# nju-websoft/MultiKE

Measured on AMD Instinct MI355X. Metric: scored triples/sec (pos+neg), higher is better.
Workload: dtype f32; 1 GPU; relation-view train step, C2-synth |E|=200000 |R|=550 dim=75 neg=25 batch=5000; n_ent=200000, n_rel=550, dim=75, neg=25, batch=5000, steps_per_epoch=184

## Files before the change

include/multike_hip.h:

```cpp
#ifndef MULTIKE_HIP_H
#define MULTIKE_HIP_H

#include <stdint.h>

#ifdef __cplusplus
extern "C" {
#endif

#define MKE_VERSION 106

#define MKE_OK 0
#define MKE_E_NULL (-1)
#define MKE_E_SHAPE (-2)
#define MKE_E_UNSUPPORTED (-3)
#define MKE_E_RANGE (-4)

#define MKE_LOSS_PARTIALS 2048

#define MKE_MAX_STRIDE 320

#define MKE_OPT_ADAGRAD 0
#define MKE_OPT_SGD 1
#define MKE_OPT_ADAM 2
#define MKE_OPT_ADADELTA 3
// ... 113 lines not shown
int mke_rows_update_multi_count(const mke_update_table* tables, int n_tables, int32_t tag, int stride, int dim,
                                int optimizer, float lr, const mke_count_job* count , void* stream);

typedef struct mke_kg_side {
  const int32_t* ent_list;
  int32_t ent_lo;
  int32_t n_ent;
  const int32_t* cand_table;
  const uint8_t* cand_valid;
  int32_t cand_k;
  const uint64_t* known_keys;
  uint64_t known_capacity;
} mke_kg_side;

int mke_neg_sample(
    const int32_t* pos_h, const int32_t* pos_r, const int32_t* pos_t, int64_t n_pos, int64_t pos_offset,
    const uint8_t* pos_kg , const mke_kg_side* sides ,
    int neg_per_pos, int max_try,
    uint32_t seed_lo, uint32_t seed_hi, uint32_t stream_id,
    int32_t* neg_h, int32_t* neg_r, int32_t* neg_t,
    void* stream);
int mke_neg_sample_at(
    const int32_t* pos_h, const int32_t* pos_r, const int32_t* pos_t, int64_t n_pos, const int32_t* pos_index,
    const uint8_t* pos_kg , const mke_kg_side* sides ,
    int neg_per_pos, int max_try,
    uint32_t seed_lo, uint32_t seed_hi, uint32_t stream_id,
    int32_t* neg_h, int32_t* neg_r, int32_t* neg_t,
    void* stream);

int mke_tripleset_build(
    const int32_t* h, const int32_t* r, const int32_t* t, int64_t n,
    uint64_t* keys, uint64_t capacity, void* stream);

int mke_tripleset_query(
    const int32_t* h, const int32_t* r, const int32_t* t, int64_t n,
    const uint64_t* keys, uint64_t capacity, uint8_t* out, void* stream);

int mke_sample_distinct(int64_t n, int batch, int n_steps, uint32_t seed_lo, uint32_t seed_hi, uint32_t stream_id,
                        int32_t* out , void* stream);

int mke_gathered_logistic_fwd_bwd(
    const float* hs, const float* rs, const float* ts, const float* ws ,
    int64_t n, int dim, int ld, int sign,
    float* gh, float* gr, float* gt,
    double* loss_partials ,
    void* stream);

int mke_gathered_alignment_fwd_bwd(
    const float* a, const float* b, int64_t n, int dim, int ld,
    float* ga, float* gb,
    double* loss_partials, void* stream);

int mke_align_fwd_bwd(
    const float* table_a, int a_normalize, const float* table_b, int b_normalize,
    int stride, int dim,
    const int32_t* ia, const int32_t* ib, int64_t n,
    float weight,
    float* grad_a , int32_t* touched_a, float* grad_b , int32_t* touched_b,
    int32_t tag,
    double* loss_partials, void* stream);

#define MKE_ALIGN_MAX_TABLES 4
#define MKE_ALIGN_MAX_TERMS 4
typedef struct mke_align_table {
  float* table; float* acc ; float* grad ; int32_t* touched;
  int64_t n_rows; int normalize;
} mke_align_table;
typedef struct mke_align_term { int a, b; float weight; } mke_align_term;
typedef struct mke_align_plan {
  mke_align_table tables[MKE_ALIGN_MAX_TABLES]; int n_tables;
  mke_align_term terms[MKE_ALIGN_MAX_TERMS]; int n_terms;
  int stride, dim;
// ... 323 lines not shown
```

multike_amd/_lib.py:

```python
from __future__ import annotations

import ctypes as C
import os

import numpy as np
import torch

_HERE = os.path.dirname(os.path.abspath(__file__))
SO_PATH = os.path.join(_HERE, "libmultike_hip.so")

LOSS_PARTIALS = 2048
MAX_STRIDE = 320
OPT_ADAGRAD, OPT_SGD, OPT_ADAM, OPT_ADADELTA = 0, 1, 2, 3
DENSE_OPTS = {"Adam": OPT_ADAM, "Adadelta": OPT_ADADELTA}
_SUPPORTED_FPL = (1, 2, 3, 4, 5, 6, 7, 8, 10, 12, 13, 16, 20)

SYMBOLS = (
    "mke_version", "mke_last_error", "mke_set_option", "mke_triple_score_fwd_bwd", "mke_triple_score_fwd_bwd_x",
    "mke_count_entity_refs", "mke_triple_score_fwd_bwd_xc", "mke_triple_score_fwd_bwd_xch", "mke_triple_score_fwd_bwd_det", "mke_stage_reduce", "mke_rows_update", "mke_rows_update_multi", "mke_rows_update_multi_count",
    "mke_neg_sample", "mke_tripleset_build", "mke_tripleset_query", "mke_gathered_logistic_fwd_bwd",
    "mke_gathered_alignment_fwd_bwd", "mke_align_fwd_bwd", "mke_gather_rows", "mke_relation_steps",
    "mke_rowset_build", "mke_rowset_remap", "mke_rows_gather_padded", "mke_rows_scatter_add",
    "mke_attr_conv_fwd", "mke_attr_conv_bwd", "mke_attr_tail_z", "mke_attr_tail_loss", "mke_attr_tail_bwd",
    "mke_dense_update", "mke_align_rank", "mke_gemm_f32", "mke_attr_scratch_floats", "mke_attr_step", "mke_attr_steps", "mke_attr_step_phases",
    "mke_sample_distinct", "mke_neg_sample_at", "mke_rows_update_dense", "mke_dense_update_opt", "mke_align_steps", "mke_sim_select", "mke_sim_sample", "mke_topk_rows", "mke_topk_candidates", "mke_mapping_scratch_floats", "mke_mapping_step", "mke_mapping_step_phases", "mke_mapping_steps",
    "mke_ae_scratch_floats", "mke_ae_train_steps", "mke_ae_step_phases", "mke_ae_encode", "mke_dense_layer_fwd",
    "mke_topk_long", "mke_probe_rows", "mke_oc_block_floats", "mke_oc_pack_codes", "mke_oc_plan", "mke_oc_bases", "mke_oc_count", "mke_oc_score", "mke_oc_apply", "mke_oc_run",
    "mke_oc_em_plan_temp_bytes", "mke_oc_em_plan", "mke_oc_pass2", "mke_oc_steps",
    "mke_tuning_init", "mke_triple_score_fwd_bwd_t", "mke_rows_update_multi_t",
    "mke_align_topk_mean_temp_bytes", "mke_align_topk_mean", "mke_align_rank_ex",
)
ACT_NONE, ACT_TANH, ACT_SIGMOID = 0, 1, 2
AE_MAX_LAYERS = 4


class AttrStepArgs(C.Structure):
    _fields_ = [
        ("ent_table", C.c_void_p), ("n_ent", C.c_int64), ("ent_stride", C.c_int), ("ent_normalize", C.c_int),
        ("ent_acc", C.c_void_p), ("ent_grad", C.c_void_p), ("ent_touched", C.c_void_p),
        ("attr_table", C.c_void_p), ("n_attr", C.c_int64), ("attr_stride", C.c_int), ("attr_normalize", C.c_int),
        ("attr_acc", C.c_void_p), ("attr_grad", C.c_void_p), ("attr_touched", C.c_void_p),
        ("lit_table", C.c_void_p), ("lit_stride", C.c_int), ("dim", C.c_int),
        ("ih", C.c_void_p), ("ia", C.c_void_p), ("iv", C.c_void_p), ("weights", C.c_void_p), ("n", C.c_int64),
        ("scale", C.c_float), ("params", C.c_void_p), ("param_grads", C.c_void_p), ("param_acc", C.c_void_p),
        ("scratch", C.c_void_p), ("partials", C.c_void_p), ("optimizer", C.c_int), ("lr", C.c_float), ("tag", C.c_int32),
        ("update", C.c_int), ("workspace", C.c_void_p), ("attr_grad_copies", C.c_int), ("tuning", C.c_void_p),
    ]


class AlignTableStruct(C.Structure):
    _fields_ = [("table", C.c_void_p), ("acc", C.c_void_p), ("grad", C.c_void_p), ("touched", C.c_void_p), ("n_rows", C.c_int64),
                ("normalize", C.c_int)]


class AlignTermStruct(C.Structure):
    _fields_ = [("a", C.c_int), ("b", C.c_int), ("weight", C.c_float)]


class AlignPlanStruct(C.Structure):
    _fields_ = [("tables", AlignTableStruct * 4), ("n_tables", C.c_int), ("terms", AlignTermStruct * 4), ("n_terms", C.c_int),
                ("stride", C.c_int), ("dim", C.c_int), ("ia", C.c_void_p), ("ib", C.c_void_p),
                ("step_off", C.POINTER(C.c_int64)), ("n_steps", C.c_int), ("optimizer", C.c_int), ("lr", C.c_float),
                ("tag_base", C.c_int32), ("loss_partials", C.c_void_p)]
# ... 133 lines not shown
        ("neg_per_pos", C.c_int), ("max_try", C.c_int), ("sample_chunk", C.c_int), ("negatives_ready", C.c_int),
        ("neg_h", C.c_void_p), ("neg_r", C.c_void_p), ("neg_t", C.c_void_p),
        ("seed_lo", C.c_uint32), ("seed_hi", C.c_uint32), ("stream_id", C.c_uint32),
        ("optimizer", C.c_int), ("lr", C.c_float), ("scale", C.c_float),
        ("loss_partials", C.c_void_p), ("loss_ring", C.c_int), ("tag_base", C.c_int32), ("pos_w", C.c_void_p),
        ("hot", HotRowsStruct), ("tuning", C.c_void_p),
    ]

_lib = None


class MultiKEHipError(RuntimeError):
    pass


def lib():
    global _lib
    if _lib is None:
        if not os.path.exists(SO_PATH):
            raise MultiKEHipError(
                f"{SO_PATH} not found: build it with `python -c 'import __graft_entry__ as g; g.build()'` "
                "or `make -C multike_amd/csrc`.  multike_amd has no CPU fallback.")
        L = C.CDLL(SO_PATH)
        L.mke_version.restype = C.c_int
        L.mke_last_error.restype = C.c_char_p
        for name in SYMBOLS[2:]:
            getattr(L, name).restype = C.c_int
        L.mke_attr_scratch_floats.restype = C.c_int64
        L.mke_mapping_scratch_floats.restype = C.c_int64
        L.mke_ae_scratch_floats.restype = C.c_int64
        L.mke_oc_block_floats.restype = C.c_int64
        L.mke_oc_em_plan_temp_bytes.restype = C.c_int64
        L.mke_align_topk_mean_temp_bytes.restype = C.c_int64
        _lib = L
        for kv in filter(None, os.environ.get("MKE_OPTIONS", "").split(",")):
            k, _, v = kv.partition("=")
            if L.mke_set_option(k.strip().encode(), C.c_int(int(v)), None):
                raise MultiKEHipError(f"MKE_OPTIONS: {L.mke_last_error().decode()}")
    return _lib


def stride_for(dim: int) -> int:
    need = (dim + 15) // 16
    for f in _SUPPORTED_FPL:
        if f >= need:
            return f * 16
    raise MultiKEHipError(f"dim {dim} exceeds the largest supported stride {MAX_STRIDE}")


def _check(rc: int, what: str):
    if rc != 0:
        msg = lib().mke_last_error().decode("utf-8", "replace")
        raise MultiKEHipError(f"{what} failed (code {rc}): {msg}")


def _dev(t: torch.Tensor | None, dtype, name: str):
    if t is None:
        return C.c_void_p(0)
    if not t.is_cuda:
        raise MultiKEHipError(f"{name}: expected a CUDA/HIP tensor, got device {t.device} (no CPU path exists)")
    if t.dtype != dtype:
        raise MultiKEHipError(f"{name}: expected dtype {dtype}, got {t.dtype}")
    if not t.is_contiguous():
        raise MultiKEHipError(f"{name}: tensor must be contiguous")
    return C.c_void_p(t.data_ptr())

# ... 294 lines not shown
    rc = lib().mke_mapping_step_phases(C.byref(args), _dev(loss_partials, torch.float64, "loss_partials"), C.c_int(phases), _stream())
    _check(rc, "mke_mapping_step_phases")


def mapping_step(args: MappingStepArgs, loss_partials: torch.Tensor):
    rc = lib().mke_mapping_step(C.byref(args), _dev(loss_partials, torch.float64, "loss_partials"), _stream())
    _check(rc, "mke_mapping_step")


def mapping_steps(args: MappingStepArgs, step_off: np.ndarray, loss_ring: torch.Tensor):
    off = np.ascontiguousarray(step_off, dtype=np.int64)
    rc = lib().mke_mapping_steps(C.byref(args), off.ctypes.data_as(C.POINTER(C.c_int64)), C.c_int(len(off) - 1),
                                 _dev(loss_ring, torch.float64, "loss_ring"), C.c_int(loss_ring.shape[0]), _stream())
    _check(rc, "mke_mapping_steps")


def align_steps(plan: AlignPlanStruct):
    rc = lib().mke_align_steps(C.byref(plan), _stream())
    _check(rc, "mke_align_steps")


def relation_steps(plan: RelationPlanStruct, step_begin: int, step_end: int):
    rc = lib().mke_relation_steps(C.byref(plan), C.c_int(step_begin), C.c_int(step_end), _stream())
    _check(rc, "mke_relation_steps")


def tripleset_build(h, r, t, keys):
    rc = lib().mke_tripleset_build(_dev(h, torch.int32, "h"), _dev(r, torch.int32, "r"), _dev(t, torch.int32, "t"),
                                   C.c_int64(h.numel()), _dev(keys, torch.int64, "keys"), C.c_uint64(keys.numel()),
                                   _stream())
    _check(rc, "mke_tripleset_build")


def tripleset_query(h, r, t, keys, out):
    rc = lib().mke_tripleset_query(_dev(h, torch.int32, "h"), _dev(r, torch.int32, "r"), _dev(t, torch.int32, "t"),
                                   C.c_int64(h.numel()), _dev(keys, torch.int64, "keys"), C.c_uint64(keys.numel()),
                                   _dev(out, torch.uint8, "out"), _stream())
    _check(rc, "mke_tripleset_query")


def gathered_logistic_fwd_bwd(hs, rs, ts, ws, sign, gh, gr, gt, loss_partials):
    n, dim = hs.shape
    rc = lib().mke_gathered_logistic_fwd_bwd(
        _dev(hs, torch.float32, "hs"), _dev(rs, torch.float32, "rs"), _dev(ts, torch.float32, "ts"),
        _dev(ws, torch.float32, "ws"), C.c_int64(n), C.c_int(dim), C.c_int(dim), C.c_int(sign),
        _dev(gh, torch.float32, "gh"), _dev(gr, torch.float32, "gr"), _dev(gt, torch.float32, "gt"),
        _dev(loss_partials, torch.float64, "loss_partials"), _stream())
    _check(rc, "mke_gathered_logistic_fwd_bwd")


def gathered_alignment_fwd_bwd(a, b, ga, gb, loss_partials):
    n, dim = a.shape
    rc = lib().mke_gathered_alignment_fwd_bwd(
        _dev(a, torch.float32, "a"), _dev(b, torch.float32, "b"), C.c_int64(n), C.c_int(dim), C.c_int(dim),
        _dev(ga, torch.float32, "ga"), _dev(gb, torch.float32, "gb"),
        _dev(loss_partials, torch.float64, "loss_partials"), _stream())
    _check(rc, "mke_gathered_alignment_fwd_bwd")


def align_fwd_bwd(table_a, a_normalize, table_b, b_normalize, dim, ia, ib, weight, grad_a, touched_a, grad_b, touched_b,
                  tag, loss_partials):
    rc = lib().mke_align_fwd_bwd(
        _dev(table_a, torch.float32, "table_a"), C.c_int(int(a_normalize)), _dev(table_b, torch.float32, "table_b"),
        C.c_int(int(b_normalize)), C.c_int(table_a.shape[1]), C.c_int(dim), _dev(ia, torch.int32, "ia"),
        _dev(ib, torch.int32, "ib"), C.c_int64(ia.numel()), C.c_float(weight), _dev(grad_a, torch.float32, "grad_a"),
        _dev(touched_a, torch.int32, "touched_a"), _dev(grad_b, torch.float32, "grad_b"),
# ... 360 lines not shown
```

multike_amd/csrc/mke_sampler.hip:

```cpp
#include "mke_common.h"

namespace mke {

struct SampleParams {
  const int32_t* __restrict__ ph;
  const int32_t* __restrict__ pr;
  const int32_t* __restrict__ pt;
  const uint8_t* __restrict__ pos_kg;
  int64_t n_pos, pos_offset;
  const int32_t* __restrict__ pos_index;
  int npp, max_try;
  mke_kg_side side[2];
  uint32_t seed_lo, seed_hi, sid;
  int32_t* __restrict__ nh;
  int32_t* __restrict__ nr;
  int32_t* __restrict__ nt;
};

__host__ __device__ __forceinline__ uint32_t draw_next(uint32_t gi, uint32_t round, uint32_t slot, uint32_t sid,
                                                       uint32_t k0, uint32_t k1, uint32_t n, uint32_t& attempt) {
  for (;;) {
    const uint32_t blk = attempt >> 2, word = attempt & 3u;
    const Philox4 ph = philox4x32_10(gi, round | (blk << 8), slot, sid, k0, k1);
    const uint32_t x = ph.v[word];
    ++attempt;
    const uint64_t m = (uint64_t)x * (uint64_t)n;
    const uint32_t l = (uint32_t)m;
    if (l < n) {
      const uint32_t thresh = (0u - n) % n;
      if (l < thresh) continue;
    }
    return (uint32_t)(m >> 32);
  }
}

__device__ __forceinline__ bool set_contains(const uint64_t* __restrict__ keys, uint64_t cap, uint64_t key) {
  uint64_t slot = mix64(key) & (cap - 1);
  for (;;) {
    const uint64_t k = keys[slot];
    if (k == key) return true;
    if (k == MKE_EMPTY_KEY) return false;
    slot = (slot + 1) & (cap - 1);
  }
}

template <int GS, bool FAST>
__global__ __launch_bounds__(MKE_BLOCK) void k_neg_sample(const SampleParams p) {
  constexpr int PPW = 64 / GS;
  constexpr int TS = 2 * GS;
  __shared__ uint32_t s_dup[FAST ? (MKE_BLOCK / GS) * TS : 1];
  const int lane = threadIdx.x & 63;
  const int gl = lane & (GS - 1);
  const int gbase = lane & ~(GS - 1);
  const int64_t wave = ((int64_t)blockIdx.x * MKE_BLOCK + threadIdx.x) >> 6;
  const int64_t i = wave * PPW + (lane / GS);
  const bool live = i < p.n_pos;
  const int64_t ii = live ? i : 0;
  const int h = p.ph[ii], r = p.pr[ii], t = p.pt[ii];
  const int kg = p.pos_kg ? (p.pos_kg[ii] != 0) : 0;
  const mke_kg_side& sd = p.side[kg];
  const uint32_t sid = p.sid + (uint32_t)kg;
  const uint64_t* __restrict__ keys = sd.known_keys;
  const uint32_t gi = p.pos_index ? (uint32_t)p.pos_index[ii] : (uint32_t)(ii + p.pos_offset);
  const int N = p.npp;
  const uint64_t gmask_all = GS == 64 ? ~0ull : (((1ull << (GS & 63)) - 1ull) << gbase);
  int collected = live ? 0 : N;
  for (int round = 0; round < p.max_try; ++round) {
    if (!__ballot(collected < N)) break;
    const int need = N - collected;
    const bool active = gl < need;
    const bool merged = FAST && N < GS;
    bool corrupt_head;
    uint32_t first_word = 0;
    if (merged) {
      const Philox4 ph = philox4x32_10(gi, (uint32_t)round, gl == GS - 1 ? 0xFFFFFFFFu : (uint32_t)gl, sid, p.seed_lo, p.seed_hi);
      first_word = ph.v[0];
      corrupt_head = ((uint32_t)__shfl((int)ph.v[0], gbase + GS - 1, 64) >> 31) != 0;
    } else {
      const Philox4 cph = philox4x32_10(gi, (uint32_t)round, 0xFFFFFFFFu, sid, p.seed_lo, p.seed_hi);
      corrupt_head = (cph.v[0] >> 31) != 0;
    }
    const int x = corrupt_head ? h : t;
    const bool use_tbl = sd.cand_table != nullptr && (sd.cand_valid == nullptr || sd.cand_valid[x] != 0);
    const uint32_t n = use_tbl ? (uint32_t)sd.cand_k : (uint32_t)sd.n_ent;
    uint32_t attempt = 0;
    uint32_t pos = 0xFFFFFFFFu;
    if (active) {
      bool have = false;
      if (merged) {
        attempt = 1;
        const uint64_t m = (uint64_t)first_word * (uint64_t)n;
        const uint32_t l = (uint32_t)m;
        have = l >= n || l >= (0u - n) % n;
        pos = (uint32_t)(m >> 32);
      }
// ... 11 lines not shown
        for (;;) {
          const uint32_t old = atomicCAS(&tbl[sl], 0xFFFFFFFFu, pos);
          if (old == 0xFFFFFFFFu) break;
          if (old == pos) { dup = true; break; }
          sl = (sl + 1) & (TS - 1);
        }
      }
    } else {
      for (int q = 0; q < need_max; ++q) {
        const uint32_t v = (uint32_t)__shfl((int)pos, gbase + q, 64);
        dup |= active && q < need && gl > q && pos == v;
      }
    }
    if (__ballot(dup)) {
      for (int q = 1; q < need_max; ++q) {
        for (;;) {
          const uint32_t v = (uint32_t)__shfl((int)pos, gbase + q, 64);
          const bool hit = q < need && gl < q && pos == v;
          const uint64_t hb = __ballot(hit);
          if (!hb) break;
          if ((hb & gmask_all) && gl == q) pos = draw_next(gi, (uint32_t)round, (uint32_t)gl, sid, p.seed_lo, p.seed_hi, n, attempt);
        }
      }
    }
    int ent = 0;
    if (active) {
      ent = use_tbl ? sd.cand_table[(int64_t)x * sd.cand_k + pos]
                    : (sd.ent_list ? sd.ent_list[pos] : sd.ent_lo + (int32_t)pos);
    }
    const int nh = corrupt_head ? ent : h;
    const int nt = corrupt_head ? t : ent;
    bool keep = active;
    if (active && round < p.max_try - 1 && keys != nullptr) {
      keep = !set_contains(keys, sd.known_capacity, triple_key((uint32_t)nh, (uint32_t)r, (uint32_t)nt));
    }
    const uint64_t mask = (__ballot(keep) & gmask_all) >> gbase;
    if (keep) {
      const int rank = __popcll(mask & ((1ull << gl) - 1ull));
      const int64_t o = i * (int64_t)N + collected + rank;
      p.nh[o] = nh; p.nr[o] = r; p.nt[o] = nt;
    }
    collected += __popcll(mask);
  }
}

__global__ __launch_bounds__(MKE_BLOCK) void k_tripleset_build(const int32_t* __restrict__ h, const int32_t* __restrict__ r,
                                                               const int32_t* __restrict__ t, int64_t n,
                                                               uint64_t* __restrict__ keys, uint64_t cap) {
  const int64_t i = (int64_t)blockIdx.x * MKE_BLOCK + threadIdx.x;
  if (i >= n) return;
  const uint64_t key = triple_key((uint32_t)h[i], (uint32_t)r[i], (uint32_t)t[i]);
  uint64_t slot = mix64(key) & (cap - 1);
  for (;;) {
    const unsigned long long prev =
        atomicCAS((unsigned long long*)&keys[slot], (unsigned long long)MKE_EMPTY_KEY, (unsigned long long)key);
    if (prev == MKE_EMPTY_KEY || prev == key) return;
    slot = (slot + 1) & (cap - 1);
  }
}

__global__ __launch_bounds__(MKE_BLOCK) void k_tripleset_query(const int32_t* __restrict__ h, const int32_t* __restrict__ r,
                                                               const int32_t* __restrict__ t, int64_t n,
                                                               const uint64_t* __restrict__ keys, uint64_t cap,
                                                               uint8_t* __restrict__ out) {
  const int64_t i = (int64_t)blockIdx.x * MKE_BLOCK + threadIdx.x;
  if (i >= n) return;
  out[i] = set_contains(keys, cap, triple_key((uint32_t)h[i], (uint32_t)r[i], (uint32_t)t[i])) ? 1 : 0;
}

}

namespace mke {
int validate_side(const mke_kg_side& sd, int neg_per_pos) {
  if (sd.n_ent < neg_per_pos) { set_error("candidate population (%d) smaller than neg_per_pos (%d)", sd.n_ent, neg_per_pos); return MKE_E_SHAPE; }
  if (sd.cand_table && sd.cand_k < neg_per_pos) { set_error("neighbour list (%d) shorter than neg_per_pos (%d)", sd.cand_k, neg_per_pos); return MKE_E_SHAPE; }
  if (sd.known_keys && (sd.known_capacity == 0 || (sd.known_capacity & (sd.known_capacity - 1)) != 0)) { set_error("known_capacity must be a power of two"); return MKE_E_SHAPE; }
  return MKE_OK;
}

int launch_neg_sample(const int32_t* pos_h, const int32_t* pos_r, const int32_t* pos_t, int64_t n_pos, int64_t pos_offset,
                      const int32_t* pos_index,
                      const uint8_t* pos_kg, const mke_kg_side* sides, int neg_per_pos, int max_try, uint32_t seed_lo,
                      uint32_t seed_hi, uint32_t stream_id, int32_t* neg_h, int32_t* neg_r, int32_t* neg_t, hipStream_t st) {
  SampleParams p;
  p.ph = pos_h; p.pr = pos_r; p.pt = pos_t; p.pos_kg = pos_kg; p.n_pos = n_pos; p.pos_offset = pos_offset; p.pos_index = pos_index;
  p.npp = neg_per_pos; p.max_try = max_try;
  p.side[0] = sides[0];
  p.side[1] = pos_kg ? sides[1] : sides[0];
  p.seed_lo = seed_lo; p.seed_hi = seed_hi; p.sid = stream_id;
  p.nh = neg_h; p.nr = neg_r; p.nt = neg_t;
  const int gs = (tune_sampler_fast() && neg_per_pos <= 15) ? 16 : (neg_per_pos <= 32 ? 32 : 64);
  const int64_t pos_per_block = (MKE_BLOCK / 64) * (64 / gs);
  const int64_t blocks = (n_pos + pos_per_block - 1) / pos_per_block;
  const dim3 grid((unsigned)blocks), blk(MKE_BLOCK);
  if (tune_sampler_fast()) {
    if (gs == 16) hipLaunchKernelGGL((k_neg_sample<16, true>), grid, blk, 0, st, p);
    else if (gs == 32) hipLaunchKernelGGL((k_neg_sample<32, true>), grid, blk, 0, st, p);
    else hipLaunchKernelGGL((k_neg_sample<64, true>), grid, blk, 0, st, p);
  } else {
    if (gs == 32) hipLaunchKernelGGL((k_neg_sample<32, false>), grid, blk, 0, st, p);
    else hipLaunchKernelGGL((k_neg_sample<64, false>), grid, blk, 0, st, p);
  }
  return check_launch("k_neg_sample");
}

__host__ __device__ __forceinline__ uint32_t feistel_round_fn(uint32_t x, uint32_t key) {
  x = x * 0x9E3779B1u + key;
  x ^= x >> 15; x *= 0x85EBCA6Bu;
  x ^= x >> 13; x *= 0xC2B2AE35u;
  x ^= x >> 16;
  return x;
}

__global__ __launch_bounds__(MKE_BLOCK) void k_sample_distinct(uint32_t n, int batch, int n_steps, uint32_t seed_lo, uint32_t seed_hi,
                                                               uint32_t stream_id, int half_bits, int32_t* __restrict__ out) {
  const int step = blockIdx.y;
  const Philox4 ka = philox4x32_10((uint32_t)step, 0u, 0x5A4D504Cu, stream_id, seed_lo, seed_hi);
  const Philox4 kb = philox4x32_10((uint32_t)step, 1u, 0x5A4D504Cu, stream_id, seed_lo, seed_hi);
  const uint32_t keys[6] = {ka.v[0], ka.v[1], ka.v[2], ka.v[3], kb.v[0], kb.v[1]};
  const uint32_t mask = (1u << half_bits) - 1u;
  for (int i = blockIdx.x * MKE_BLOCK + threadIdx.x; i < batch; i += gridDim.x * MKE_BLOCK) {
// ... 29 lines not shown
    if (rc) return rc;
  }
  return launch_neg_sample(pos_h, pos_r, pos_t, n_pos, pos_offset, pos_index, pos_kg, sides, neg_per_pos, max_try, seed_lo, seed_hi,
                           stream_id, neg_h, neg_r, neg_t, (hipStream_t)stream);
}

extern "C" int mke_neg_sample(const int32_t* pos_h, const int32_t* pos_r, const int32_t* pos_t, int64_t n_pos,
                              int64_t pos_offset, const uint8_t* pos_kg, const mke_kg_side* sides, int neg_per_pos,
                              int max_try, uint32_t seed_lo, uint32_t seed_hi, uint32_t stream_id, int32_t* neg_h,
                              int32_t* neg_r, int32_t* neg_t, void* stream) {
  return neg_sample_checked(pos_h, pos_r, pos_t, n_pos, pos_offset, nullptr, pos_kg, sides, neg_per_pos, max_try, seed_lo, seed_hi,
                            stream_id, neg_h, neg_r, neg_t, stream);
}

extern "C" int mke_neg_sample_at(const int32_t* pos_h, const int32_t* pos_r, const int32_t* pos_t, int64_t n_pos,
                                 const int32_t* pos_index, const uint8_t* pos_kg, const mke_kg_side* sides, int neg_per_pos,
                                 int max_try, uint32_t seed_lo, uint32_t seed_hi, uint32_t stream_id, int32_t* neg_h,
                                 int32_t* neg_r, int32_t* neg_t, void* stream) {
  if (n_pos > 0 && !pos_index) { mke::set_error("mke_neg_sample_at: NULL pos_index"); return MKE_E_NULL; }
  return neg_sample_checked(pos_h, pos_r, pos_t, n_pos, 0, pos_index, pos_kg, sides, neg_per_pos, max_try, seed_lo, seed_hi,
                            stream_id, neg_h, neg_r, neg_t, stream);
}

extern "C" int mke_tripleset_build(const int32_t* h, const int32_t* r, const int32_t* t, int64_t n, uint64_t* keys,
                                   uint64_t capacity, void* stream) {
  using namespace mke;
  if (n < 0) { set_error("negative n"); return MKE_E_SHAPE; }
  if (n == 0) return MKE_OK;
  if (!h || !r || !t || !keys) { set_error("mke_tripleset_build: NULL pointer"); return MKE_E_NULL; }
  if (capacity == 0 || (capacity & (capacity - 1)) != 0 || capacity < (uint64_t)n + 1) {
    set_error("capacity must be a power of two > n");
    return MKE_E_SHAPE;
  }
  const int64_t blocks = (n + MKE_BLOCK - 1) / MKE_BLOCK;
  hipLaunchKernelGGL(k_tripleset_build, dim3((unsigned)blocks), dim3(MKE_BLOCK), 0, (hipStream_t)stream, h, r, t, n,
                     keys, capacity);
  return check_launch("k_tripleset_build");
}

extern "C" int mke_tripleset_query(const int32_t* h, const int32_t* r, const int32_t* t, int64_t n,
                                   const uint64_t* keys, uint64_t capacity, uint8_t* out, void* stream) {
  using namespace mke;
  if (n < 0) { set_error("negative n"); return MKE_E_SHAPE; }
  if (n == 0) return MKE_OK;
  if (!h || !r || !t || !keys || !out) { set_error("mke_tripleset_query: NULL pointer"); return MKE_E_NULL; }
  if (capacity == 0 || (capacity & (capacity - 1)) != 0) { set_error("capacity must be a power of two"); return MKE_E_SHAPE; }
  const int64_t blocks = (n + MKE_BLOCK - 1) / MKE_BLOCK;
  hipLaunchKernelGGL(k_tripleset_query, dim3((unsigned)blocks), dim3(MKE_BLOCK), 0, (hipStream_t)stream, h, r, t, n,
                     keys, capacity, out);
  return check_launch("k_tripleset_query");
}

extern "C" int mke_sample_distinct(int64_t n, int batch, int n_steps, uint32_t seed_lo, uint32_t seed_hi, uint32_t stream_id,
                                   int32_t* out, void* stream) {
  using namespace mke;
  if (n < 0 || batch < 0 || n_steps < 0 || n > 0x7FFFFFFFLL || (int64_t)batch > n) { set_error("mke_sample_distinct: need 0 <= batch <= n < 2^31 (n=%lld batch=%d)", (long long)n, batch); return MKE_E_SHAPE; }
  if (batch == 0 || n_steps == 0) return MKE_OK;
  if (!out) { set_error("mke_sample_distinct: NULL output"); return MKE_E_NULL; }
  if (n_steps > 65535) { set_error("mke_sample_distinct: more than 65535 steps"); return MKE_E_SHAPE; }
  int half = 1;
  while ((1ll << (2 * half)) < n) ++half;
  int bx = (batch + MKE_BLOCK - 1) / MKE_BLOCK;
  if (bx > 64) bx = 64;
  hipLaunchKernelGGL(k_sample_distinct, dim3(bx, n_steps), dim3(MKE_BLOCK), 0, (hipStream_t)stream, (uint32_t)n, batch, n_steps, seed_lo,
                     seed_hi, stream_id, half, out);
  return check_launch("k_sample_distinct");
}
```

multike_amd/sampling.py:

```python
from __future__ import annotations

import math

import numpy as np
import torch

from . import _lib


def kg_batch_split(n1: int, n2: int, batch_size: int):
    b1 = int(n1 / (n1 + n2) * batch_size)
    return b1, batch_size - b1


class KnownTripleSet:

    MAX_ENT, MAX_REL = (1 << 26) - 1, 1 << 12

    def __init__(self, h: torch.Tensor, r: torch.Tensor, t: torch.Tensor):
        n = h.numel()
        if n and (int(h.max()) >= self.MAX_ENT or int(t.max()) >= self.MAX_ENT or int(r.max()) >= self.MAX_REL):
            raise _lib.MultiKEHipError("entity id >= 2^26 - 1 or relation id >= 2^12 does not fit the packed triple key")
        cap = 1
        while cap < 2 * n + 2:
            cap *= 2
        self.keys = torch.full((cap,), -1, dtype=torch.int64, device=h.device)
        self.add(h, r, t)

    def add(self, h, r, t):
        _lib.tripleset_build(h.contiguous(), r.contiguous(), t.contiguous(), self.keys)

    def contains(self, h, r, t) -> torch.Tensor:
        out = torch.empty(h.numel(), dtype=torch.uint8, device=h.device)
        _lib.tripleset_query(h.contiguous(), r.contiguous(), t.contiguous(), self.keys, out)
        return out.bool()


class KGSide:

    def __init__(self, entities, known: KnownTripleSet | None, device="cuda"):
        ents = np.asarray(entities, dtype=np.int64)
        self.n_ent = len(ents)
        if self.n_ent and np.array_equal(ents, np.arange(ents[0], ents[0] + self.n_ent)):
            self.ent_lo, self.ent_list = int(ents[0]), None
        else:
            self.ent_lo, self.ent_list = 0, torch.as_tensor(ents, dtype=torch.int32, device=device)
        self.known = known
        self.cand_table = None
        self.cand_valid = None

    def set_neighbours(self, cand_table: torch.Tensor | None, cand_valid: torch.Tensor | None):
        self.cand_table, self.cand_valid = cand_table, cand_valid

    def fill(self, st: "_lib.KGSideStruct"):
        st.ent_list = _lib.ptr(self.ent_list, torch.int32, "ent_list")
        st.ent_lo, st.n_ent = self.ent_lo, self.n_ent
        st.cand_table = _lib.ptr(self.cand_table, torch.int32, "cand_table")
        st.cand_valid = _lib.ptr(self.cand_valid, torch.uint8, "cand_valid")
        st.cand_k = 0 if self.cand_table is None else self.cand_table.shape[1]
        st.known_keys = None if self.known is None else _lib.ptr(self.known.keys, torch.int64, "known_keys")
        st.known_capacity = 0 if self.known is None else self.known.keys.numel()


# ... 2 lines not shown
    side0.fill(arr[0])
    (side1 or side0).fill(arr[1])
    return arr


def sample_negatives(pos, side: KGSide, neg_per_pos: int, seed=(0, 0), stream_id=0, pos_offset=0, max_try=10,
                     out=None, side1: KGSide | None = None, pos_kg: torch.Tensor | None = None):
    ph, pr, pt = pos
    n = ph.numel() * neg_per_pos
    if out is None:
        out = tuple(torch.empty(n, dtype=torch.int32, device=ph.device) for _ in range(3))
    if n:
        _lib.neg_sample(pos, pos_offset, pos_kg, side_array(side, side1), neg_per_pos, max_try, seed, stream_id, out)
    return out


def int_triples(triples) -> np.ndarray:
    if isinstance(triples, np.ndarray) or hasattr(triples, "__array__"):
        return np.asarray(triples, dtype=np.int32).reshape(-1, 3)
    if hasattr(triples, "cols"):
        return np.asarray(triples.cols, dtype=np.int32).reshape(-1, 3)
    import itertools
    n = len(triples)
    if n == 0:
        return np.zeros((0, 3), dtype=np.int32)
    first = next(iter(triples))
    if len(first) != 3:
        return np.asarray(list(triples), dtype=np.int32).reshape(-1, 3)
    return np.fromiter(itertools.chain.from_iterable(triples), dtype=np.int64, count=3 * n).reshape(n, 3).astype(np.int32)


class RelationBatcher:

    def __init__(self, triples1, triples2, side1: KGSide, side2: KGSide, batch_size: int, neg_per_pos: int,
                 device="cuda", seed: int = 0):
        self.device = torch.device(device)
        self.t1 = torch.as_tensor(int_triples(triples1), device=self.device)
        self.t2 = torch.as_tensor(int_triples(triples2), device=self.device)
        self.side1, self.side2 = side1, side2
        self.batch_size, self.neg_per_pos = int(batch_size), int(neg_per_pos)
        self.n1, self.n2 = self.t1.shape[0], self.t2.shape[0]
        self.b1, self.b2 = kg_batch_split(self.n1, self.n2, self.batch_size)
        self.steps = int(math.ceil((self.n1 + self.n2) / self.batch_size))
        self.seed = int(seed)
        self.epoch = 0
        self._gen = torch.Generator(device=self.device)
        self._gen.manual_seed(self.seed)
        self._layout()
        self._materialise(None, None)

    def _layout(self):
        s = np.arange(self.steps, dtype=np.int64)
        self.lo1, self.hi1 = np.minimum(s * self.b1, self.n1), np.minimum((s + 1) * self.b1, self.n1)
        self.lo2, self.hi2 = np.minimum(s * self.b2, self.n2), np.minimum((s + 1) * self.b2, self.n2)
        c1, c2 = self.hi1 - self.lo1, self.hi2 - self.lo2
        self.off = np.zeros(self.steps + 1, dtype=np.int64)
        self.off[1:] = np.cumsum(c1 + c2)
        self.cnt1 = c1
        src = np.empty(int(self.off[-1]), dtype=np.int64)
        for i in range(self.steps):
            o = self.off[i]
            src[o:o + c1[i]] = np.arange(self.lo1[i], self.hi1[i])
            src[o + c1[i]:self.off[i + 1]] = self.n1 + np.arange(self.lo2[i], self.hi2[i])
        self._src = torch.as_tensor(src, device=self.device)
        kg = np.zeros(int(self.off[-1]), dtype=np.uint8)
        for i in range(self.steps):
            kg[self.off[i] + c1[i]:self.off[i + 1]] = 1
        self.pos_kg = torch.as_tensor(kg, device=self.device)

    def _materialise(self, perm1, perm2):
        if self.device.type == "cuda":
            cur = torch.cuda.current_stream(self.device)
            for t in (self.t1, self.t2):
                t.record_stream(cur)
        t1 = self.t1 if perm1 is None else self.t1[perm1]
        t2 = self.t2 if perm2 is None else self.t2[perm2]
        allt = torch.cat([t1, t2], 0)[self._src]
        if getattr(self, "pos_h", None) is None:
            self.pos_h = allt[:, 0].contiguous()
            self.pos_r = allt[:, 1].contiguous()
            self.pos_t = allt[:, 2].contiguous()
        else:
            self.pos_h.copy_(allt[:, 0])
            self.pos_r.copy_(allt[:, 1])
            self.pos_t.copy_(allt[:, 2])
        self.t1, self.t2 = t1, t2

    def stage_next_epoch(self):
        p1 = torch.randperm(self.n1, generator=self._gen, device=self.device)
        p2 = torch.randperm(self.n2, generator=self._gen, device=self.device)
        t1, t2 = self.t1[p1], self.t2[p2]
        allt = torch.cat([t1, t2], 0)[self._src]
        if getattr(self, "_alt", None) is None:
            self._alt = tuple(allt[:, k].contiguous() for k in range(3))
        else:
            for k in range(3):
                self._alt[k].copy_(allt[:, k])
        self._staged_lists = (t1, t2)
        return self._alt

    def commit_staged(self):
        cur = (self.pos_h, self.pos_r, self.pos_t)
        self.pos_h, self.pos_r, self.pos_t = self._alt
        self._alt = cur
        self.t1, self.t2 = self._staged_lists
        self._staged_lists = None
        self.epoch += 1

    def shuffle(self):
        p1 = torch.randperm(self.n1, generator=self._gen, device=self.device)
        p2 = torch.randperm(self.n2, generator=self._gen, device=self.device)
        self._materialise(p1, p2)
        self.epoch += 1

    def positives(self, step: int):
        lo, hi = int(self.off[step]), int(self.off[step + 1])
        return self.pos_h[lo:hi], self.pos_r[lo:hi], self.pos_t[lo:hi]

    @property
    def rng_seed(self):
        return (self.seed & 0xFFFFFFFF, (self.seed >> 32) & 0xFFFFFFFF)

    @property
    def rng_stream(self):
        return (self.epoch * 2) & 0xFFFFFFFF

    def batch(self, step: int, out=None):
        lo, hi = int(self.off[step]), int(self.off[step + 1])
        N = self.neg_per_pos
        if out is None:
            out = tuple(torch.empty((hi - lo) * N, dtype=torch.int32, device=self.device) for _ in range(3))
        pos = (self.pos_h[lo:hi], self.pos_r[lo:hi], self.pos_t[lo:hi])
        if hi > lo:
            sample_negatives(pos, self.side1, N, seed=self.rng_seed, stream_id=self.rng_stream, pos_offset=lo, out=out,
                             side1=self.side2, pos_kg=self.pos_kg[lo:hi])
        return pos, out
```

Before: 2.227 billion triples/s.

## Add bitmap prefilter for known-triple lookups, fused epoch positives kernel, prefetched perms

Builds a per-table bit filter alongside the known-triple hash set so the negative sampler can skip most hash probes when the filter bit is clear. Adds a single kernel that applies the epoch permutations and scatters positives into the per-step layout, replacing several torch gather, cat and copy ops. Random permutations for the next epoch are drawn ahead of time on a side stream. This adds a host-side global registry keyed by pointer, which carries lifetime and staleness risks. Filter memory is capped at 2^25 bits.

Measured after the change: 2.289 billion triples/s, median of 6. 1.03x the previous value.

```diff
diff --git a/include/multike_hip.h b/include/multike_hip.h
--- a/include/multike_hip.h
+++ b/include/multike_hip.h
@@ -169,12 +169,20 @@
     const int32_t* h, const int32_t* r, const int32_t* t, int64_t n,
     uint64_t* keys, uint64_t capacity, void* stream);
 
+int mke_tripleset_forget(const uint64_t* keys);
+int64_t mke_tripleset_filter_bytes(const uint64_t* keys, uint64_t capacity);
+
 int mke_tripleset_query(
     const int32_t* h, const int32_t* r, const int32_t* t, int64_t n,
     const uint64_t* keys, uint64_t capacity, uint8_t* out, void* stream);
 
 int mke_sample_distinct(int64_t n, int batch, int n_steps, uint32_t seed_lo, uint32_t seed_hi, uint32_t stream_id,
                         int32_t* out , void* stream);
+
+int mke_epoch_positives(const int32_t* list1, const int32_t* list2, int64_t n1, int64_t n2, const int64_t* perm1 ,
+                        const int64_t* perm2 , int64_t b1, int64_t b2, int64_t n_steps,
+                        int32_t* list1_out , int32_t* list2_out ,
+                        int32_t* pos_h, int32_t* pos_r, int32_t* pos_t, void* stream);
 
 int mke_gathered_logistic_fwd_bwd(
     const float* hs, const float* rs, const float* ts, const float* ws ,
diff --git a/multike_amd/_lib.py b/multike_amd/_lib.py
--- a/multike_amd/_lib.py
+++ b/multike_amd/_lib.py
@@ -29,6 +29,7 @@
     "mke_oc_em_plan_temp_bytes", "mke_oc_em_plan", "mke_oc_pass2", "mke_oc_steps",
     "mke_tuning_init", "mke_triple_score_fwd_bwd_t", "mke_rows_update_multi_t",
     "mke_align_topk_mean_temp_bytes", "mke_align_topk_mean", "mke_align_rank_ex",
+    "mke_tripleset_forget", "mke_tripleset_filter_bytes", "mke_epoch_positives",
 )
 ACT_NONE, ACT_TANH, ACT_SIGMOID = 0, 1, 2
 AE_MAX_LAYERS = 4
@@ -228,6 +229,7 @@
         L.mke_oc_block_floats.restype = C.c_int64
         L.mke_oc_em_plan_temp_bytes.restype = C.c_int64
         L.mke_align_topk_mean_temp_bytes.restype = C.c_int64
+        L.mke_tripleset_filter_bytes.restype = C.c_int64
         _lib = L
         for kv in filter(None, os.environ.get("MKE_OPTIONS", "").split(",")):
             k, _, v = kv.partition("=")
@@ -588,6 +590,35 @@
     _check(rc, "mke_tripleset_build")
 
 
+def tripleset_forget(keys):
+    addr = keys if isinstance(keys, int) else keys.data_ptr()
+    _check(lib().mke_tripleset_forget(C.c_void_p(addr)), "mke_tripleset_forget")
+
+
+def tripleset_filter_bytes(keys) -> int:
+    return int(lib().mke_tripleset_filter_bytes(_dev(keys, torch.int64, "keys"), C.c_uint64(keys.numel())))
+
+
+def epoch_positives(list1, list2, perm1, perm2, b1, b2, n_steps, list1_out, list2_out, pos):
+    i32, i64 = torch.int32, torch.int64
+    n1, n2 = list1.shape[0], list2.shape[0]
+    need = min(n_steps * b1, n1) + min(n_steps * b2, n2)
+    for x in pos:
+        if x.numel() < need:
+            raise MultiKEHipError(f"epoch buffers hold {x.numel()} positives, the layout needs {need}")
+    for pm, n in ((perm1, n1), (perm2, n2)):
+        if pm is not None and pm.numel() != n:
+            raise MultiKEHipError("a permutation must be as long as its list")
+    for o, l in ((list1_out, list1), (list2_out, list2)):
+        if o is not None and o.shape != l.shape:
+            raise MultiKEHipError("a shuffled list must have its list's shape")
+    rc = lib().mke_epoch_positives(_dev(list1, i32, "list1"), _dev(list2, i32, "list2"), C.c_int64(n1), C.c_int64(n2),
+                                   _dev(perm1, i64, "perm1"), _dev(perm2, i64, "perm2"), C.c_int64(b1), C.c_int64(b2),
+                                   C.c_int64(n_steps), _dev(list1_out, i32, "list1_out"), _dev(list2_out, i32, "list2_out"),
+                                   _dev(pos[0], i32, "pos_h"), _dev(pos[1], i32, "pos_r"), _dev(pos[2], i32, "pos_t"), _stream())
+    _check(rc, "mke_epoch_positives")
+
+
 def tripleset_query(h, r, t, keys, out):
     rc = lib().mke_tripleset_query(_dev(h, torch.int32, "h"), _dev(r, torch.int32, "r"), _dev(t, torch.int32, "t"),
                                    C.c_int64(h.numel()), _dev(keys, torch.int64, "keys"), C.c_uint64(keys.numel()),
diff --git a/multike_amd/csrc/mke_epoch.hip b/multike_amd/csrc/mke_epoch.hip
--- /dev/null
+++ b/multike_amd/csrc/mke_epoch.hip
@@ -0,0 +1,57 @@
+#include "mke_common.h"
+
+namespace mke {
+
+struct EpochParams {
+  const int32_t* __restrict__ list_in[2];
+  int32_t* __restrict__ list_out[2];
+  const int64_t* __restrict__ perm[2];
+  int64_t n[2];
+  int64_t b[2];
+  int64_t n_steps;
+  int32_t* __restrict__ pos_h;
+  int32_t* __restrict__ pos_r;
+  int32_t* __restrict__ pos_t;
+};
+
+__global__ __launch_bounds__(MKE_BLOCK) void k_epoch_positives(const EpochParams p) {
+  int64_t i = (int64_t)blockIdx.x * MKE_BLOCK + threadIdx.x;
+  int kg = 0;
+  if (i >= p.n[0]) { i -= p.n[0]; kg = 1; }
+  if (i >= p.n[kg]) return;
+  const int64_t src = p.perm[kg] ? p.perm[kg][i] : i;
+  const int32_t* row = p.list_in[kg] + 3 * src;
+  const int32_t h = row[0], r = row[1], t = row[2];
+  if (p.list_out[kg]) {
+    int32_t* o = p.list_out[kg] + 3 * i;
+    o[0] = h; o[1] = r; o[2] = t;
+  }
+  const int64_t b = p.b[kg];
+  if (b <= 0) return;
+  const int64_t s = i / b;
+  if (s >= p.n_steps) return;
+  const int64_t before1 = min(s * p.b[0], p.n[0]), before2 = min(s * p.b[1], p.n[1]);
+  int64_t e = before1 + before2 + (i - s * b);
+  if (kg == 1) e += min((s + 1) * p.b[0], p.n[0]) - before1;
+  p.pos_h[e] = h; p.pos_r[e] = r; p.pos_t[e] = t;
+}
+
+}
+
+extern "C" int mke_epoch_positives(const int32_t* list1, const int32_t* list2, int64_t n1, int64_t n2, const int64_t* perm1,
+                                   const int64_t* perm2, int64_t b1, int64_t b2, int64_t n_steps, int32_t* list1_out,
+                                   int32_t* list2_out, int32_t* pos_h, int32_t* pos_r, int32_t* pos_t, void* stream) {
+  using namespace mke;
+  if (n1 < 0 || n2 < 0 || b1 < 0 || b2 < 0 || n_steps < 0) { set_error("mke_epoch_positives: negative count"); return MKE_E_SHAPE; }
+  if (n1 + n2 > 0x7FFFFFFFLL) { set_error("mke_epoch_positives: more than 2^31 - 1 positives"); return MKE_E_SHAPE; }
+  if (n1 + n2 == 0) return MKE_OK;
+  if ((n1 && !list1) || (n2 && !list2) || !pos_h || !pos_r || !pos_t) { set_error("mke_epoch_positives: NULL pointer"); return MKE_E_NULL; }
+  if ((list1_out && list1_out == list1) || (list2_out && list2_out == list2)) { set_error("mke_epoch_positives: a list cannot be shuffled in place"); return MKE_E_SHAPE; }
+  EpochParams p;
+  p.list_in[0] = list1; p.list_in[1] = list2; p.list_out[0] = list1_out; p.list_out[1] = list2_out;
+  p.perm[0] = perm1; p.perm[1] = perm2; p.n[0] = n1; p.n[1] = n2; p.b[0] = b1; p.b[1] = b2; p.n_steps = n_steps;
+  p.pos_h = pos_h; p.pos_r = pos_r; p.pos_t = pos_t;
+  const int64_t blocks = (n1 + n2 + MKE_BLOCK - 1) / MKE_BLOCK;
+  hipLaunchKernelGGL(k_epoch_positives, dim3((unsigned)blocks), dim3(MKE_BLOCK), 0, (hipStream_t)stream, p);
+  return check_launch("k_epoch_positives");
+}
diff --git a/multike_amd/csrc/mke_sampler.hip b/multike_amd/csrc/mke_sampler.hip
--- a/multike_amd/csrc/mke_sampler.hip
+++ b/multike_amd/csrc/mke_sampler.hip
@@ -1,6 +1,13 @@
+#include <mutex>
+#include <unordered_map>
+
 #include "mke_common.h"
 
 namespace mke {
+
+constexpr int FILTER_BITS_PER_SLOT_LOG2 = 3;
+constexpr int FILTER_MAX_BITS_LOG2 = 25;
+constexpr int FILTER_MIN_BITS_LOG2 = 10;
 
 struct SampleParams {
   const int32_t* __restrict__ ph;
@@ -11,6 +18,8 @@
   const int32_t* __restrict__ pos_index;
   int npp, max_try;
   mke_kg_side side[2];
+  const uint32_t* __restrict__ filter[2];
+  int filter_shift[2];
   uint32_t seed_lo, seed_hi, sid;
   int32_t* __restrict__ nh;
   int32_t* __restrict__ nr;
@@ -34,14 +43,21 @@
   }
 }
 
-__device__ __forceinline__ bool set_contains(const uint64_t* __restrict__ keys, uint64_t cap, uint64_t key) {
-  uint64_t slot = mix64(key) & (cap - 1);
+__device__ __forceinline__ bool set_contains_hashed(const uint64_t* __restrict__ keys, uint64_t cap, uint64_t key, uint64_t hash) {
+  uint64_t slot = hash & (cap - 1);
   for (;;) {
     const uint64_t k = keys[slot];
     if (k == key) return true;
     if (k == MKE_EMPTY_KEY) return false;
     slot = (slot + 1) & (cap - 1);
   }
+}
+__device__ __forceinline__ bool set_contains(const uint64_t* __restrict__ keys, uint64_t cap, uint64_t key) {
+  return set_contains_hashed(keys, cap, key, mix64(key));
+}
+__device__ __forceinline__ bool filter_maybe(const uint32_t* __restrict__ filter, int shift, uint64_t hash) {
+  const uint64_t bit = hash >> shift;
+  return (filter[bit >> 5] >> (uint32_t)(bit & 31u)) & 1u;
 }
 
 template <int GS, bool FAST>
@@ -61,6 +77,8 @@
   const mke_kg_side& sd = p.side[kg];
   const uint32_t sid = p.sid + (uint32_t)kg;
   const uint64_t* __restrict__ keys = sd.known_keys;
+  const uint32_t* __restrict__ filter = p.filter[kg];
+  const int fshift = p.filter_shift[kg];
   const uint32_t gi = p.pos_index ? (uint32_t)p.pos_index[ii] : (uint32_t)(ii + p.pos_offset);
   const int N = p.npp;
   const uint64_t gmask_all = GS == 64 ? ~0ull : (((1ull << (GS & 63)) - 1ull) << gbase);
@@ -138,7 +156,9 @@
     const int nt = corrupt_head ? t : ent;
     bool keep = active;
     if (active && round < p.max_try - 1 && keys != nullptr) {
-      keep = !set_contains(keys, sd.known_capacity, triple_key((uint32_t)nh, (uint32_t)r, (uint32_t)nt));
+      const uint64_t key = triple_key((uint32_t)nh, (uint32_t)r, (uint32_t)nt);
+      const uint64_t hash = mix64(key);
+      if (filter == nullptr || filter_maybe(filter, fshift, hash)) keep = !set_contains_hashed(keys, sd.known_capacity, key, hash);
     }
     const uint64_t mask = (__ballot(keep) & gmask_all) >> gbase;
     if (keep) {
@@ -152,11 +172,17 @@
 
 __global__ __launch_bounds__(MKE_BLOCK) void k_tripleset_build(const int32_t* __restrict__ h, const int32_t* __restrict__ r,
                                                                const int32_t* __restrict__ t, int64_t n,
-                                                               uint64_t* __restrict__ keys, uint64_t cap) {
+                                                               uint64_t* __restrict__ keys, uint64_t cap,
+                                                               uint32_t* __restrict__ filter, int filter_shift) {
   const int64_t i = (int64_t)blockIdx.x * MKE_BLOCK + threadIdx.x;
   if (i >= n) return;
   const uint64_t key = triple_key((uint32_t)h[i], (uint32_t)r[i], (uint32_t)t[i]);
-  uint64_t slot = mix64(key) & (cap - 1);
+  const uint64_t hash = mix64(key);
+  if (filter) {
+    const uint64_t bit = hash >> filter_shift;
+    atomicOr(&filter[bit >> 5], 1u << (uint32_t)(bit & 31u));
+  }
+  uint64_t slot = hash & (cap - 1);
   for (;;) {
     const unsigned long long prev =
         atomicCAS((unsigned long long*)&keys[slot], (unsigned long long)MKE_EMPTY_KEY, (unsigned long long)key);
@@ -172,6 +198,81 @@
   const int64_t i = (int64_t)blockIdx.x * MKE_BLOCK + threadIdx.x;
   if (i >= n) return;
   out[i] = set_contains(keys, cap, triple_key((uint32_t)h[i], (uint32_t)r[i], (uint32_t)t[i])) ? 1 : 0;
+}
+
+__global__ __launch_bounds__(MKE_BLOCK) void k_filter_from_table(const uint64_t* __restrict__ keys, uint64_t cap,
+                                                                 uint32_t* __restrict__ filter, int filter_shift) {
+  const uint64_t i = (uint64_t)blockIdx.x * MKE_BLOCK + threadIdx.x;
+  if (i >= cap) return;
+  const uint64_t key = keys[i];
+  if (key == MKE_EMPTY_KEY) return;
+  const uint64_t bit = mix64(key) >> filter_shift;
+  atomicOr(&filter[bit >> 5], 1u << (uint32_t)(bit & 31u));
+}
+
+struct TripleFilter {
+  uint64_t capacity;
+  uint32_t* bits;
+  int shift;
+};
+static std::mutex g_filter_mu;
+static std::unordered_map<const void*, TripleFilter> g_filters;
+
+static int filter_bits_log2(uint64_t capacity) {
+  int lg = 0;
+  while ((1ull << lg) < capacity) ++lg;
+  lg += FILTER_BITS_PER_SLOT_LOG2;
+  return lg < FILTER_MIN_BITS_LOG2 ? FILTER_MIN_BITS_LOG2 : (lg > FILTER_MAX_BITS_LOG2 ? FILTER_MAX_BITS_LOG2 : lg);
+}
+
+static TripleFilter filter_lookup(const uint64_t* keys, uint64_t capacity) {
+  std::lock_guard<std::mutex> lk(g_filter_mu);
+  const auto it = g_filters.find(keys);
+  if (it == g_filters.end() || it->second.capacity != capacity) return TripleFilter{0, nullptr, 0};
+  return it->second;
+}
+
+static void filter_forget(const void* keys) {
+  std::lock_guard<std::mutex> lk(g_filter_mu);
+  const auto it = g_filters.find(keys);
+  if (it == g_filters.end()) return;
+  (void)hipFree(it->second.bits);
+  g_filters.erase(it);
+}
+
+static int filter_for_build(uint64_t* keys, uint64_t capacity, hipStream_t st, TripleFilter* out) {
+  std::lock_guard<std::mutex> lk(g_filter_mu);
+  auto it = g_filters.find(keys);
+  if (it != g_filters.end() && it->second.capacity != capacity) {
+    (void)hipFree(it->second.bits);
+    g_filters.erase(it);
+    it = g_filters.end();
+  }
+  if (it != g_filters.end()) { *out = it->second; return MKE_OK; }
+  const int lg = filter_bits_log2(capacity);
+  const size_t bytes = (size_t)1 << (lg - 3);
+  int cur = 0, dev = 0;
+  hipPointerAttribute_t attr;
+  if (hipGetDevice(&cur) != hipSuccess) { set_error("mke_tripleset_build: no device"); return MKE_E_NULL; }
+  dev = cur;
+  if (hipPointerGetAttributes(&attr, keys) == hipSuccess) dev = attr.device; else (void)hipGetLastError();
+  TripleFilter f{capacity, nullptr, 64 - lg};
+  if (dev != cur) (void)hipSetDevice(dev);
+  hipError_t e = hipMalloc((void**)&f.bits, bytes);
+  if (e == hipSuccess) e = hipMemsetAsync(f.bits, 0, bytes, st);
+  if (dev != cur) (void)hipSetDevice(cur);
+  if (e != hipSuccess) {
+    if (f.bits) (void)hipFree(f.bits);
+    set_error("mke_tripleset_build: filter allocation (%zu bytes): %s", bytes, hipGetErrorString(e));
+    return (int)e;
+  }
+  const uint64_t blocks = (capacity + MKE_BLOCK - 1) / MKE_BLOCK;
+  hipLaunchKernelGGL(k_filter_from_table, dim3((unsigned)blocks), dim3(MKE_BLOCK), 0, st, keys, capacity, f.bits, f.shift);
+  const int rc = check_launch("k_filter_from_table");
+  if (rc) { (void)hipFree(f.bits); return rc; }
+  g_filters.emplace(keys, f);
+  *out = f;
+  return MKE_OK;
 }
 
 }
@@ -193,6 +294,11 @@
   p.npp = neg_per_pos; p.max_try = max_try;
   p.side[0] = sides[0];
   p.side[1] = pos_kg ? sides[1] : sides[0];
+  for (int k = 0; k < 2; ++k) {
+    const TripleFilter f = p.side[k].known_keys ? filter_lookup(p.side[k].known_keys, p.side[k].known_capacity) : TripleFilter{0, nullptr, 0};
+    p.filter[k] = f.bits;
+    p.filter_shift[k] = f.shift;
+  }
   p.seed_lo = seed_lo; p.seed_hi = seed_hi; p.sid = stream_id;
   p.nh = neg_h; p.nr = neg_r; p.nt = neg_t;
   const int gs = (tune_sampler_fast() && neg_per_pos <= 15) ? 16 : (neg_per_pos <= 32 ? 32 : 64);
@@ -288,10 +394,23 @@
     set_error("capacity must be a power of two > n");
     return MKE_E_SHAPE;
   }
+  TripleFilter f;
+  const int rc = filter_for_build(keys, capacity, (hipStream_t)stream, &f);
+  if (rc) return rc;
   const int64_t blocks = (n + MKE_BLOCK - 1) / MKE_BLOCK;
   hipLaunchKernelGGL(k_tripleset_build, dim3((unsigned)blocks), dim3(MKE_BLOCK), 0, (hipStream_t)stream, h, r, t, n,
-                     keys, capacity);
+                     keys, capacity, f.bits, f.shift);
   return check_launch("k_tripleset_build");
+}
+
+extern "C" int64_t mke_tripleset_filter_bytes(const uint64_t* keys, uint64_t capacity) {
+  const mke::TripleFilter f = keys ? mke::filter_lookup(keys, capacity) : mke::TripleFilter{0, nullptr, 0};
+  return f.bits ? (int64_t)1 << (64 - f.shift - 3) : 0;
+}
+
+extern "C" int mke_tripleset_forget(const uint64_t* keys) {
+  if (keys) mke::filter_forget(keys);
+  return MKE_OK;
 }
 
 extern "C" int mke_tripleset_query(const int32_t* h, const int32_t* r, const int32_t* t, int64_t n,
diff --git a/multike_amd/sampling.py b/multike_amd/sampling.py
--- a/multike_amd/sampling.py
+++ b/multike_amd/sampling.py
@@ -25,10 +25,20 @@
         while cap < 2 * n + 2:
             cap *= 2
         self.keys = torch.full((cap,), -1, dtype=torch.int64, device=h.device)
+        self._addr = self.keys.data_ptr() if self.keys.is_cuda else None
+        if self._addr is not None:
+            _lib.tripleset_forget(self._addr)
         self.add(h, r, t)
 
     def add(self, h, r, t):
         _lib.tripleset_build(h.contiguous(), r.contiguous(), t.contiguous(), self.keys)
+
+    def __del__(self):
+        try:
+            if getattr(self, "_addr", None) is not None:
+                _lib.tripleset_forget(self._addr)
+        except Exception:
+            pass
 
     def contains(self, h, r, t) -> torch.Tensor:
         out = torch.empty(h.numel(), dtype=torch.uint8, device=h.device)
@@ -97,8 +107,10 @@
 
 class RelationBatcher:
 
+    PREFETCH_PERMS = True
+
     def __init__(self, triples1, triples2, side1: KGSide, side2: KGSide, batch_size: int, neg_per_pos: int,
-                 device="cuda", seed: int = 0):
+                 device="cuda", seed: int = 0, prefetch_perms: bool | None = None):
         self.device = torch.device(device)
         self.t1 = torch.as_tensor(int_triples(triples1), device=self.device)
         self.t2 = torch.as_tensor(int_triples(triples2), device=self.device)
@@ -111,7 +123,14 @@
         self.epoch = 0
         self._gen = torch.Generator(device=self.device)
         self._gen.manual_seed(self.seed)
+        self._native = self.device.type == "cuda"
+        self._prefetch = self._native and bool(self.PREFETCH_PERMS if prefetch_perms is None else prefetch_perms)
+        self._perm_stream = self._next_perms = None
         self._layout()
+        if self._native:
+            n_pos = int(self.off[-1])
+            self.pos_h, self.pos_r, self.pos_t = (torch.empty(n_pos, dtype=torch.int32, device=self.device) for _ in range(3))
+            self._spare_lists = (torch.empty_like(self.t1), torch.empty_like(self.t2))
         self._materialise(None, None)
 
     def _layout(self):
@@ -133,48 +152,77 @@
             kg[self.off[i] + c1[i]:self.off[i + 1]] = 1
         self.pos_kg = torch.as_tensor(kg, device=self.device)
 
-    def _materialise(self, perm1, perm2):
-        if self.device.type == "cuda":
-            cur = torch.cuda.current_stream(self.device)
-            for t in (self.t1, self.t2):
-                t.record_stream(cur)
+    def _draw_perms(self):
+        return (torch.randperm(self.n1, generator=self._gen, device=self.device),
+                torch.randperm(self.n2, generator=self._gen, device=self.device))
+
+    def _take_perms(self):
+        if not self._prefetch:
+            return self._draw_perms()
+        cur = torch.cuda.current_stream(self.device)
+        if self._perm_stream is None:
+            self._perm_stream = torch.cuda.Stream(device=self.device)
+            self._next_perms = self._draw_perms()
+        else:
+            cur.wait_stream(self._perm_stream)
+        perms = self._next_perms
+        for p in perms:
+            p.record_stream(cur)
+        with torch.cuda.stream(self._perm_stream):
+            self._next_perms = self._draw_perms()
+        return perms
+
+    def _materialise(self, perm1, perm2, staged: bool = False):
+        if self._native:
+            if staged and getattr(self, "_alt", None) is None:
+                self._alt = tuple(torch.empty_like(x) for x in (self.pos_h, self.pos_r, self.pos_t))
+            pos = self._alt if staged else (self.pos_h, self.pos_r, self.pos_t)
+            if perm1 is None:
+                _lib.epoch_positives(self.t1, self.t2, None, None, self.b1, self.b2, self.steps, None, None, pos)
+                return
+            out = self._spare_lists
+            _lib.epoch_positives(self.t1, self.t2, perm1, perm2, self.b1, self.b2, self.steps, out[0], out[1], pos)
+            if staged:
+                self._staged_lists = out
+            else:
+                self._spare_lists, (self.t1, self.t2) = (self.t1, self.t2), out
+            return
         t1 = self.t1 if perm1 is None else self.t1[perm1]
         t2 = self.t2 if perm2 is None else self.t2[perm2]
         allt = torch.cat([t1, t2], 0)[self._src]
-        if getattr(self, "pos_h", None) is None:
-            self.pos_h = allt[:, 0].contiguous()
-            self.pos_r = allt[:, 1].contiguous()
-            self.pos_t = allt[:, 2].contiguous()
+        cols = tuple(allt[:, k].contiguous() for k in range(3))
+        if staged:
+            if getattr(self, "_alt", None) is None:
+                self._alt = cols
+            else:
+                for dst, src in zip(self._alt, cols):
+                    dst.copy_(src)
+            self._staged_lists = (t1, t2)
+        elif getattr(self, "pos_h", None) is None:
+            self.pos_h, self.pos_r, self.pos_t = cols
+            self.t1, self.t2 = t1, t2
         else:
-            self.pos_h.copy_(allt[:, 0])
-            self.pos_r.copy_(allt[:, 1])
-            self.pos_t.copy_(allt[:, 2])
-        self.t1, self.t2 = t1, t2
+            for dst, src in zip((self.pos_h, self.pos_r, self.pos_t), cols):
+                dst.copy_(src)
+            self.t1, self.t2 = t1, t2
 
     def stage_next_epoch(self):
-        p1 = torch.randperm(self.n1, generator=self._gen, device=self.device)
-        p2 = torch.randperm(self.n2, generator=self._gen, device=self.device)
-        t1, t2 = self.t1[p1], self.t2[p2]
-        allt = torch.cat([t1, t2], 0)[self._src]
-        if getattr(self, "_alt", None) is None:
-            self._alt = tuple(allt[:, k].contiguous() for k in range(3))
-        else:
-            for k in range(3):
-                self._alt[k].copy_(allt[:, k])
-        self._staged_lists = (t1, t2)
+        p1, p2 = self._take_perms()
+        self._materialise(p1, p2, staged=True)
         return self._alt
 
     def commit_staged(self):
         cur = (self.pos_h, self.pos_r, self.pos_t)
         self.pos_h, self.pos_r, self.pos_t = self._alt
         self._alt = cur
+        if self._native:
+            self._spare_lists = (self.t1, self.t2)
         self.t1, self.t2 = self._staged_lists
         self._staged_lists = None
         self.epoch += 1
 
     def shuffle(self):
-        p1 = torch.randperm(self.n1, generator=self._gen, device=self.device)
-        p2 = torch.randperm(self.n2, generator=self._gen, device=self.device)
+        p1, p2 = self._take_perms()
         self._materialise(p1, p2)
         self.epoch += 1
 
```
